# programmerjake/path-trace

Hardware: AMD Instinct MI355X
Metric: Msamples/sec at 1920x1080x1024spp; per-channel RMSE vs CPU ref (higher is better)
Workload: dtype f32; 1 GPU; C3: 1920x1080, 1024 spp, depth 8, north star: 6-sphere union/difference CSG; order=fast

## Files before the change

__graft_entry__.py:

```python
import os
import sys

ROOT = os.path.dirname(os.path.abspath(__file__))
for p in (os.path.join(ROOT, "path-trace_amd"), os.path.join(ROOT, "oracle"), os.path.join(ROOT, "tests")):
    if p not in sys.path:
        sys.path.insert(0, p)


def build() -> None:
    import build_ext
    import oracle_py
    build_ext.build()
    oracle_py.build(ref=True)
    import time
    from concurrent.futures import ProcessPoolExecutor
    start = time.time() - 1
    workers = max(1, min(8, (os.cpu_count() or 1)))
    with ProcessPoolExecutor(max_workers=workers) as ex:
        list(ex.map(_compile_job, range(len(_jobs()) + len(_test_defines()))))
    from pathtrace import _lib
    from pathtrace._lib import lib
    if not _have_gpu():
        _precompile_selftest()
    _prune_cache(start)
    print("build ok:", _lib.LIB_PATH, lib().pt_version().decode())


def _jobs():
    from pathtrace.modules import product_jobs
    jobs = product_jobs()
    try:
        import precompile_modules as test_modules
    except ImportError:
        return jobs
    jobs = jobs + test_modules.test_jobs()
    try:
        import precompile_multispan as multispan_modules
    except ImportError:
        return jobs
    jobs = jobs + multispan_modules.test_jobs()
    try:
        import precompile_lane_resume as lane_resume_modules
    except ImportError:
        return jobs
    return jobs + lane_resume_modules.test_jobs()


def _compile_job(k: int) -> None:
    import pathtrace as pt
    jobs = _jobs()
    if k >= len(jobs):
        import zoo
        from precompile_modules import TEST_DEFINES
        defs, builder, depth, ls = TEST_DEFINES[k - len(jobs)]
        os.environ["PT_DEVICE_DEFINES"] = defs
        try:
            pt.DeviceScene(zoo.build(builder), lane_scatter=ls).compile(depth)
        finally:
            del os.environ["PT_DEVICE_DEFINES"]
        return
    make, depth = jobs[k]
    obj = make()
    if depth is not None:
        obj.compile(depth)


def _test_defines():
    try:
        from precompile_modules import TEST_DEFINES
    except ImportError:
        return []
    return TEST_DEFINES


CACHE = os.path.join(ROOT, "path-trace_amd", "_jit_cache")


def _prune_cache(since: float) -> None:
    if not os.path.isdir(CACHE):
        return
    for f in os.listdir(CACHE):
        if f.endswith(".hsaco") and os.path.getmtime(os.path.join(CACHE, f)) < since:
            for ext in (".hsaco", ".hip"):
                q = os.path.join(CACHE, f[:-6] + ext)
                if os.path.exists(q):
                    os.remove(q)


def _have_gpu() -> bool:
    try:
        import torch
        return torch.cuda.device_count() > 0
    except Exception:
        return False


def _precompile_selftest() -> None:
    import ctypes
    from pathtrace import _lib
    out = (ctypes.c_uint64 * 3)()
    _lib.lib().pt_selftest_math(0, 0, 0, out)


def smoke() -> None:
    import numpy as np
    import oracle_py as O
    import pathtrace as pt
    from pathtrace import scenes
    from pathtrace.scene import to_text
    W, H, spp, depth = 24, 16, 4, 8
    root = scenes.scene_p1()
    gpu = pt.render(root, W, H, spp, depth, order="fast", device=0).reshape(-1, 3)
    ref = O.render(to_text(root, "/tmp/pt_smoke_img"), W, H, spp, depth, order=O.ORDER_FAST)
    bad = int(np.sum(gpu.view(np.uint32) != ref.view(np.uint32)))
    if bad:
        raise AssertionError("smoke: %d of %d values differ from the oracle" % (bad, gpu.size))
    rmse = np.sqrt(np.mean((gpu.astype(np.float64) - ref) ** 2, axis=0))
    print("smoke ok: %dx%d x %d spp, bit-exact vs oracle, rmse %s, mean %s" % (W, H, spp, rmse, gpu.mean(axis=0)))


if __name__ == "__main__":
    if len(sys.argv) > 1 and sys.argv[1] == "smoke":
        smoke()
    else:
        build()
```

path-trace_amd/csrc/device/pt_device.h:

```cpp
#ifndef PT_DEVICE_H
#define PT_DEVICE_H

#if defined(PT_KEPT_NORM) || defined(PT_FAST_NORM) || defined(PT_FAST_MIRRORBALL) || defined(PT_UNIT_RAY) ||        \
    defined(PT_INERT) || defined(PT_PLANE_AXIS_DARK) || defined(PT_PLANE_AXIS_DIV) || defined(PT_MERGE_FROM_SPANS) || \
    defined(PT_UNION_FUSED) || defined(PT_CTX_VGPR) || defined(PT_CLEAR_UNION) || defined(PT_LSUM_LDS) ||             \
    defined(PT_RING_SPLIT) || defined(PT_LANE_MAJOR) || defined(PT_LM_CHAINS) || defined(PT_LM_BITS) ||               \
    defined(PT_RING_FITS) || defined(PT_PASS_PAIR_FALLBACK) || defined(PT_KATT_SHORT) || defined(PT_SHORT_REM) ||     \
    defined(PT_PAD_VALU) || defined(PT_PAD_SALU) || defined(PT_NO_AXIS_SHARE) || defined(PT_FAST_LANE) ||             \
    defined(PT_RECEDE_DEAD)
#error "a retired build-time knob is defined (PT_KEPT_NORM PT_FAST_NORM PT_FAST_MIRRORBALL PT_UNIT_RAY PT_INERT PT_PLANE_AXIS_DARK PT_PLANE_AXIS_DIV PT_MERGE_FROM_SPANS PT_UNION_FUSED PT_CTX_VGPR PT_CLEAR_UNION PT_LSUM_LDS PT_RING_SPLIT PT_LANE_MAJOR PT_LM_CHAINS PT_LM_BITS PT_RING_FITS PT_PASS_PAIR_FALLBACK PT_KATT_SHORT PT_SHORT_REM PT_PAD_VALU PT_PAD_SALU PT_NO_AXIS_SHARE PT_FAST_LANE PT_RECEDE_DEAD): its arm is gone, see DESIGN.md s2, Build-time knobs that remain"
#endif

typedef unsigned long long u64;
typedef unsigned int u32;

namespace ptd
{

constexpr float EPS = 1e-3f;
constexpr float MAXV = 1e20f;
constexpr u64 LCG_MULT = 214013ull;
constexpr u64 LCG_INC = 2531011ull;

struct PtImage
// ... 1118 lines not shown
                return;
            }
        }
#endif
        typename Pln<P, O, M, AX, U>::St s;
        Pln<P, O, M, AX, U>::init(s, c, q, e);
        acc.add(s.live, s.t0, s.t1, M);
    }
    __device__ static __forceinline__ void fill(float4 *, int *, const typename Pln<P, O, M, AX, U>::Ctx &) {}
};
template <class A, class B>
struct Compact<Uni<A, B>>
{
    static constexpr bool OK = Compact<A>::OK && Compact<B>::OK;
    __device__ static __forceinline__ void run(UnionAcc &acc, u64 &m, PlaneStash &st, const typename Uni<A, B>::Ctx &c,
                                               const Ray &q, const Env &e)
    {
        Compact<A>::run(acc, m, st, c.a, q, e);
        Compact<B>::run(acc, m, st, c.b, q, e);
    }
    __device__ static __forceinline__ void fill(float4 *tab, int *mt, const typename Uni<A, B>::Ctx &c)
    {
        Compact<A>::fill(tab, mt, c.a);
        Compact<B>::fill(tab, mt, c.b);
    }
};
template <class R>
__device__ __forceinline__ int compact_first_hit(const typename R::Ctx &ctx, const Ray &q, const Env &e,
                                                 const float4 *tab, const int *mt, bool &hit, float &t, int &mat)
{
    UnionAcc acc;
    u64 m = 0ull;
    PlaneStash st;
#pragma unroll
    for (int k = 0; k < 3; k++)
        st.has[k][0] = st.has[k][1] = 0;
    Compact<R>::run(acc, m, st, ctx, q, e);
#if defined(PT_AXIS_SHARE) && PT_PLANE_PAIR
    auto unit_plane = [&](int k, int side, float num, int mat) {
        const float dk = k == 0 ? q.d.x : k == 1 ? q.d.y : q.d.z;
        const float div = side ? -dk : dk;
        const bool small = __builtin_fabsf(div) < EPS * EPS;
        const float q0 = div_core(num, q.rk[k]);
        float t = side ? -q0 : q0;
        const bool bad = !small && !(q.rkok[k] && num_ok(num));
        if (wave_any(bad)) {
            if (bad)
                t = num / div;
        }
        const bool deg = small || __builtin_fabsf(t) >= MAXV;
        const bool neg = div < 0.0f;
        acc.add((!deg || __builtin_fabsf(num) < EPS * EPS) ? 1 : 0, (!deg && neg) ? t : -MAXV,
                (!deg && !neg) ? t : MAXV, mat);
    };
#pragma unroll
    for (int k = 0; k < 3; k++) {
        if (st.has[k][0] && st.has[k][1]) {
            const float dk = k == 0 ? q.d.x : k == 1 ? q.d.y : q.d.z;
            const int side = dk < 0.0f ? 0 : 1;
            unit_plane(k, side, side ? st.num[k][1] : st.num[k][0], side ? st.mat[k][1] : st.mat[k][0]);
        } else {
            if (st.has[k][0])
                unit_plane(k, 0, st.num[k][0], st.mat[k][0]);
            if (st.has[k][1])
                unit_plane(k, 1, st.num[k][1], st.mat[k][1]);
        }
    }
#endif
    while (wave_any(m != 0ull)) {
        if (m != 0ull) {
            const int k = __builtin_ctzll(m);
            m &= m - 1ull;
            const float4 sp = tab[k];
            const float b = (sp.x * q.d.x + sp.y * q.d.y) + sp.z * q.d.z;
            const float disc = b * b - q.a * sp.w;
            const float sq = sqrt_core(disc);
            const float n0 = -b - sq, n1 = -b + sq;
            float t0 = div_core(n0, q.ra), t1 = div_core(n1, q.ra);
            if (!(q.aok && num_ok(n0) && num_ok(n1)))
                t0 = n0 / q.a, t1 = n1 / q.a;
            acc.add(1, t0, t1, mt[k]);
        }
    }
    mat = acc.bm;
    t = acc.b0;
    hit = acc.found && acc.b0 < MAXV;
    return ((!acc.found) | ((acc.b0 >= EPS) & !acc.tie)) & !acc.bad;
}

#ifndef PT_OCCLUDE
#define PT_OCCLUDE 1
#endif
template <class N>
struct Occl
{
    static constexpr bool OK = false;
};
template <int P, int O, int M>
struct Occl<Sph<P, O, M>>
{
    static constexpr bool OK = true;
    template <class SEL>
    __device__ static __forceinline__ float emis_lb(const typename Sph<P, O, M>::Ctx &, const Env &)
    {
        return SEL::take(M) ? 0.0f : __builtin_inff();
    }
    template <class SEL>
    __device__ static __forceinline__ u64 occ(const typename Sph<P, O, M>::Ctx &, V3, float, const Env &)
    {
        return 0ull;
    }
};
template <int P, int O, int M, int AX, int U>
struct Occl<Pln<P, O, M, AX, U>>
{
    static constexpr bool OK = true;
    template <class SEL>
    __device__ static __forceinline__ float emis_lb(const typename Pln<P, O, M, AX, U>::Ctx &c, const Env &e)
    {
        if constexpr (!SEL::take(M))
            return __builtin_inff();
        const float nn = __builtin_sqrtf(dot(mk(e.P[O], e.P[O + 1], e.P[O + 2]), mk(e.P[O], e.P[O + 1], e.P[O + 2])));
        return c.num <= -1e-3f ? (-c.num / nn) * 0.999f : 0.0f;
    }
    template <class SEL>
    __device__ static __forceinline__ u64 occ(const typename Pln<P, O, M, AX, U>::Ctx &c, V3 w, float g, const Env &e)
    {
        if constexpr (SEL::take(M) || AX < 0) {
            return 0ull;
        } else {
            const float na = e.P[O + (AX >> 1)];
            const float wa = (AX >> 1) == 0 ? w.x : (AX >> 1) == 1 ? w.y : w.z;
            const float lim = fmaxf(1e-4f, -c.num * g);
            return __ballot(c.num <= -1e-3f && na * wa < -lim);
        }
    }
};
template <class A, class B>
struct Occl<Uni<A, B>>
{
    static constexpr bool OK = Occl<A>::OK && Occl<B>::OK;
    template <class SEL>
    __device__ static __forceinline__ float emis_lb(const typename Uni<A, B>::Ctx &c, const Env &e)
    {
        return fminf(Occl<A>::template emis_lb<SEL>(c.a, e), Occl<B>::template emis_lb<SEL>(c.b, e));
    }
    template <class SEL>
    __device__ static __forceinline__ u64 occ(const typename Uni<A, B>::Ctx &c, V3 w, float g, const Env &e)
    {
        return Occl<A>::template occ<SEL>(c.a, w, g, e) | Occl<B>::template occ<SEL>(c.b, w, g, e);
    }
};

template <class N>
struct BFlips
{
    __device__ static constexpr int of(int) { return 0; }
};
template <class A, class B>
struct BFlips<Uni<A, B>>
{
    __device__ static constexpr int of(int prim) { return prim < A::HI ? BFlips<A>::of(prim) : BFlips<B>::of(prim); }
};
template <class A, class B>
struct BFlips<Isect<A, B>>
{
    __device__ static constexpr int of(int prim) { return prim < A::HI ? BFlips<A>::of(prim) : BFlips<B>::of(prim); }
};
template <class A, class B>
struct BFlips<Diff<A, B>>
{
    __device__ static constexpr int of(int prim) { return prim < A::HI ? BFlips<A>::of(prim) : 1 + BFlips<B>::of(prim); }
};

template <int MOFF, int IOFF, class C>
struct Xf
{
    static constexpr int LO = C::LO, HI = C::HI;
    static constexpr bool UNION_ONLY = C::UNION_ONLY;
    static constexpr bool NO_DIFF = C::NO_DIFF;
    template <class PS>
    __device__ static __forceinline__ int isect_empty(const PS &ps) { return C::isect_empty(ps); }
    struct Ctx
    {
        typename C::Ctx c;
    };
    typedef typename C::St St;
    __device__ static __forceinline__ void prep(Ctx &c, V3 o, const Env &e) { C::prep(c.c, univ(m_apply(e.P + MOFF, o)), e); }
    __device__ static __forceinline__ void prep_l(Ctx &c, V3 o, const Env &e) { C::prep_l(c.c, m_apply(e.P + MOFF, o), e); }
    __device__ static __forceinline__ void init(St &s, const Ctx &c, const Ray &q, const Env &e)
    {
        C::init(s, c.c, mkray(m_lin(e.P + MOFF, q.d)), e);
    }
    __device__ static __forceinline__ bool pull(St &s, CS &out) { return C::pull(s, out); }
    template <class PS>
    __device__ static __forceinline__ void span(PS &ps, const Ctx &c, const Ray &q, const Env &e)
    {
        C::span(ps, c.c, mkray(m_lin(e.P + MOFF, q.d)), e);
    }
    template <class PS>
    __device__ static __forceinline__ void init_ps(St &s, const PS &ps) { C::init_ps(s, ps); }
    template <class F>
    __device__ static __forceinline__ void each_pos(F &&f) { C::each_pos(f); }
    template <class SEL, class PS>
    __device__ static __forceinline__ void span_sel(PS &ps, const Ctx &c, const Ray &q, const Env &e)
    {
        C::template span_sel<SEL>(ps, c.c, mkray(m_lin(e.P + MOFF, q.d)), e);
    }
    template <class SEL, class F>
    __device__ static __forceinline__ void each_sel(F &&f) { C::template each_sel<SEL>(f); }
    template <class SEL, bool NORM>
    __device__ static __forceinline__ u64 clear_mask(const Ctx &c, const Ray &q, const Env &e)
    {
        return C::template clear_mask<SEL, false>(c.c, mkray(m_lin(e.P + MOFF, q.d)), e);
    }
    template <class SEL>
    __device__ static constexpr bool clear_ok() { return C::template clear_ok<SEL>(); }
    template <class PS>
    __device__ static __forceinline__ int fast_ok(const PS &ps) { return C::fast_ok(ps); }
    __device__ static __forceinline__ V3 normal(int prim, float t, V3 o, V3 d, const Env &e)
    {
        V3 n = C::normal(prim, t, m_apply(e.P + MOFF, o), m_lin(e.P + MOFF, d), e);
        if constexpr (!C::NO_DIFF) {
            const bool neg = BFlips<C>::of(prim) & 1;
            n = neg ? -n : n;
            n = normalize(m_lin(e.P + IOFF, n));
            return neg ? -n : n;
        }
        return normalize(m_lin(e.P + IOFF, n));
    }
    template <class SEL>
    __device__ static constexpr bool raw_ok() { return C::template nsel<SEL>() == 0; }
    template <class SEL>
    __device__ static constexpr int nsel() { return C::template nsel<SEL>(); }
    template <class SEL>
    __device__ static __forceinline__ u64 dark_mask(const Ctx &, V3, const Env &) { return ~0ull; }
    template <class SEL>
    __device__ static __forceinline__ bool dark_pre(const Ctx &, const Env &) { return true; }
};
template <int MOFF, int IOFF, class C>
struct BFlips<Xf<MOFF, IOFF, C>>
{
    __device__ static constexpr int of(int prim) { return BFlips<C>::of(prim); }
};

template <class R>
__device__ __forceinline__ bool first_hit(const typename R::Ctx &ctx, V3 d, const Env &e, float &t, u32 &ref,
                                          bool &exit_hit)
{
#ifdef PT_MERGE_STUB
    (void)ctx, (void)d, (void)e, (void)t, (void)ref, (void)exit_hit;
    return false;
#endif
    typename R::St st;
    R::init(st, ctx, mkray(d), e);
    CS s;
    while (R::pull(st, s)) {
        if (s.t0 >= MAXV)
            return false;
        if (s.t0 >= EPS) {
            t = s.t0, ref = s.r0, exit_hit = false;
            return true;
        }
        if (s.t1 >= MAXV)
            return false;
        if (s.t1 >= EPS) {
            t = s.t1, ref = s.r1, exit_hit = true;
            return true;
        }
    }
    return false;
}

template <class R, class PS>
__device__ __forceinline__ bool first_hit_ps(const PS &ps, float &t, u32 &ref, bool &exit_hit)
{
    typename R::St st;
    R::init_ps(st, ps);
    CS s;
    while (R::pull(st, s)) {
        if (s.t0 >= MAXV)
            return false;
        if (s.t0 >= EPS) {
            t = s.t0, ref = s.r0, exit_hit = false;
            return true;
        }
        if (s.t1 >= MAXV)
            return false;
        if (s.t1 >= EPS) {
            t = s.t1, ref = s.r1, exit_hit = true;
            return true;
        }
    }
    return false;
}

template <class R, class PS>
__device__ __forceinline__ int cheap_ok(const PS &ps);
template <class R, class PS>
__device__ __forceinline__ int span_first_hit(const PS &ps, bool &hit, float &t, u32 &ref, bool &exit_hit)
{
    int fok;
    if constexpr (R::NO_DIFF) {
        fok = cheap_ok<R>(ps);
        if (wave_any(!fok)) {
            if (!fok)
// ... 752 lines not shown
    const W2 b1 = lcg_step(a3), b2 = lcg_step(b1), b3 = lcg_step(b2);
    s = ((u64)b3.hi << 32) | (u64)b3.lo;
    return attempt2_draws<KR0>(a1, a2, a3, b1, b2, b3, n, kR);
}
template <bool KR0>
__device__ __forceinline__ Attempt2 attempt2_draws(W2 a1, W2 a2, W2 a3, W2 b1, W2 b2, W2 b3, V3 n, V3 kR)
{
    const f2 S = 0x1p-31f, M1 = -1.0f;
    f2 x = {(float)a1.hi, (float)b1.hi}, y = {(float)a2.hi, (float)b2.hi}, z = {(float)a3.hi, (float)b3.hi};
    x = __builtin_elementwise_fma(x, S, M1);
    y = __builtin_elementwise_fma(y, S, M1);
    z = __builtin_elementwise_fma(z, S, M1);
    const f2 vv = (x * x + y * y) + z * z;
    if (!KR0) {
        x = x + kR.x;
        y = y + kR.y;
        z = z + kR.z;
    }
#ifndef PT_HEMI_MODE
#define PT_HEMI_MODE 1
#endif
#if PT_HEMI_MODE == 1
    const f2 nw = {(n.x * x.x + n.y * y.x) + n.z * z.x, (n.x * x.y + n.y * y.y) + n.z * z.y};
#elif PT_HEMI_MODE == 2
    float vnx, vny, vnz;
    asm("v_mov_b32 %0, %1" : "=v"(vnx) : "s"(n.x));
    asm("v_mov_b32 %0, %1" : "=v"(vny) : "s"(n.y));
    asm("v_mov_b32 %0, %1" : "=v"(vnz) : "s"(n.z));
    const f2 nw = (x * vnx + y * vny) + z * vnz;
#else
    const f2 nw = (x * n.x + y * n.y) + z * n.z;
#endif
    Attempt2 r;
    r.x = x, r.y = y, r.z = z;
    const bool ba = !(vv.x > 0x1.000002p+0f), bb = !(vv.y > 0x1.000002p+0f);
    const bool ha = !(nw.x <= EPS), hb = !(nw.y <= EPS);
    const u64 BA = __ballot(ba), HA = __ballot(ha), BBm = __ballot(bb), HBm = __ballot(hb);
    r.A[0] = BA & HA, r.F[0] = BA & ~HA, r.acc[0] = ba && ha;
    r.A[1] = BBm & HBm, r.F[1] = BBm & ~HBm, r.acc[1] = bb && hb;
    return r;
}

__device__ __forceinline__ int replay(u64 A, u64 F, u64 NL, int rem, int &fails, int &reason, u64 &take)
{
    const int pa = __popcll(A), pf = __popcll(F);
    if (NL == 0ull && pa < rem && fails + pf < 1000) {
        take = A;
        if (A) {
            const int last = 63 - __builtin_clzll(A);
            fails = (last == 63) ? 0 : __popcll(F >> (last + 1));
        } else {
            fails += pf;
        }
        return 63;
    }
    const int nl = NL ? __builtin_ctzll(NL) : 64;
    const int pos_rem = (pa >= rem) ? nth_set_bit(A, rem) : 64;
    int pos_abort = 64;
    if (fails + pf >= 1000) {
        int fc = fails;
        for (int l = 0; l < 64; l++) {
            if (l == nl || l == pos_rem)
                break;
            if ((A >> l) & 1ull)
                fc = 0;
            else if ((F >> l) & 1ull) {
                if (++fc == 1000) {
                    pos_abort = l;
                    break;
                }
            }
        }
    }
    if (pos_abort < 64 && pos_abort < nl && pos_abort < pos_rem) {
        reason = B_ABORT;
        take = A & ((1ull << pos_abort) - 1ull);
        return pos_abort;
    }
    if (nl < 64 && nl <= pos_rem) {
        reason = B_NONLEAF;
        take = A & ((1ull << nl) - 1ull);
        return nl;
    }
    if (pos_rem < 64) {
        reason = B_DONE;
        take = (pos_rem == 63) ? A : (A & ((2ull << pos_rem) - 1ull));
        return pos_rem;
    }
    take = A;
    if (A) {
        const int last = 63 - __builtin_clzll(A);
        fails = (last == 63) ? 0 : __popcll(F >> (last + 1));
    } else {
        fails += pf;
    }
    return 63;
}

template <class S, bool STRICT, bool DEFERRED, bool KR0>
__device__ __forceinline__ int burst_t(const Env &e, Rng &rng, const u64 *__restrict__ jump, const JumpLds &J,
                                       const WaveLds &L, Frame &f, Frame &child, Counters &cnt)
{
    float4 *const ring = L.ring;
    unsigned char *const slowq = L.slowq, *const midq = L.midq;
    constexpr bool LANE_REMAT = PT_LANE_REMAT < 0 ? S::Root::NO_DIFF : PT_LANE_REMAT != 0;
    const int lane_reg = threadIdx.x & 63;
#define lane (LANE_REMAT ? lane_id() : lane_reg)
    const bool LSUM_LDS = L.lsum != nullptr;
    const V3 hit = univ(f.hit), n = univ(f.n), rc = univ(f.rc);
    const float sc = unif(f.sc), strength = unif(f.strength), add = unif(f.add);
    const int depth = uni(f.depth), N = uni(f.N);
    const int i = uni(f.i);
    V3 retval = univ(f.retval);
    const V3 kR = univ((1.0f / sc - 1.0f) * univ(f.refl));
    const float sNa = unif((strength / (float)N) * add);
    const float aN = unif(add / (float)N);
    const float abs_rc = unif(length(rc));
    const bool child_leaf_depth = depth - 1 <= 0;
    auto lane_state = [&]() {
        u64 jA, jG;
        jread(J.j3, lane, jA, jG);
        return jA * rng.st + jG;
    };
    const u64 A64 = jump[128], g64inc = jump[129] * LCG_INC;
    const u64 Afull = jump[128 * PT_KATT], gfullinc = jump[128 * PT_KATT + 1] * LCG_INC;
    int fails = 0, reason = -1;
    LdsBox<typename S::Root::Ctx> *const cxp = (LdsBox<typename S::Root::Ctx> *)L.ctx;
    typename S::Root::Ctx c0;
    S::Root::prep(c0, hit, e);
    lds_put(*cxp, c0);
    if constexpr (PT_SPH_COMPACT && Compact<typename S::Root>::OK)
        Compact<typename S::Root>::fill(L.stab, L.smat, c0);
    int npos = 0, nkeep = 0, keep_sum = 0, nzc = 0, f_n = 0, s_head = 0, s_n = 0, s_first = 0;
    int m_head = 0, m_n = 0, m_first = 0;
    V3 lsum = mk(0.0f, 0.0f, 0.0f);
    if (LSUM_LDS)
        L.lsum[lane] = L.lsum[64 + lane] = L.lsum[128 + lane] = 0.0f;
    int fast_on = 1, clear_on = 1;
    constexpr bool CLEAR = S::Root::template clear_ok<Emissive<S>>() && !S::Root::UNION_ONLY;
    constexpr bool RAW = DEFERRED && !STRICT && S::Root::template raw_ok<Emissive<S>>();
    const bool wfin = __builtin_fabsf(rc.x) < 1e37f && __builtin_fabsf(rc.y) < 1e37f && __builtin_fabsf(rc.z) < 1e37f;
    const u64 raw_mask =
        uni_mask((KR0 || length(kR) < 64.0f) && wfin && S::Root::template dark_pre<Emissive<S>>(c0, e));
#if PT_OCCLUDE
    constexpr bool OCC = RAW && Occl<typename S::Root>::OK;
#else
    constexpr bool OCC = false;
#endif
    float occ_g = __builtin_inff();
    if constexpr (OCC) {
        const float te = fminf(Occl<typename S::Root>::template emis_lb<Emissive<S>>(c0, e), 1e19f);
        const float bw = (KR0 ? 1.0f : 1.0f + length(kR)) * 1.0001f;
        occ_g = unif(te > 0.0f ? bw * 1.001f / te : __builtin_inff());
    }
    auto dark = [&](V3 wn) -> u64 {
        u64 d = S::Root::template dark_mask<Emissive<S>>(c0, wn, e);
        if constexpr (OCC)
            d |= Occl<typename S::Root>::template occ<Emissive<S>>(c0, wn, occ_g, e);
        return d & raw_mask;
    };
    const bool short_nd = !DEFERRED && EPS < 0.99f * (sNa * abs_rc);
    auto slot_pos = [&](unsigned char v) { return keep_sum + ((int)(v - keep_sum) & (PT_RCAP - 1)); };
    PT_CNT(cnt, 0, 1);
    for (;;) {
        PT_CNT(cnt, 1, 1);
        const bool room = PT_RCAP - (nkeep - keep_sum) >= 64;
        if (reason < 0 && room) {
            PT_T0(tg);
            PT_MARK(13);
            int rem = N - (i + npos);
            const int katt = (rem <= 24 || (!DEFERRED && short_nd)) ? PT_KATT : PT_KATT;
            int free_slots = PT_RCAP - (nkeep - keep_sum);
#ifdef PT_ROOM_CAP
            free_slots = min(free_slots, PT_ROOM_CAP);
#endif
            int ta = 0, tk = 0;
            u64 nlor = 0ull, Alast = 0ull, Flast = 0ull;
            const int slot_end = nkeep + free_slots;
            auto write_attempt = [&](u64 A, u64 kp, V3 wn, float factor) {
                const int slot = mbcnt(kp, nkeep + tk);
                if (in_mask(kp & __ballot(slot < slot_end)))
                    ring[slot & (PT_RCAP - 1)] = make_float4(wn.x, wn.y, wn.z, factor);
                ta += __popcll(A);
                tk += __popcll(kp);
            };
            int fails_lm = 0;
            if constexpr (DEFERRED) {
                u64 jA, jG;
                jread(J.j24, lane, jA, jG);
                const u64 s_lane = jA * rng.st + jG;
                u32 abits = 0u, fbits = 0u, kbits = 0u;
                u64 sk = s_lane;
#pragma unroll
                for (int k = 0; k < PT_KATT; k += 2) {
                    const Attempt2 ap = attempt2_chain<KR0>(sk, n, kR);
#pragma unroll
                    for (int h = 0; h < 2; h++) {
                        const V3 wn = h ? mk(ap.x.y, ap.y.y, ap.z.y) : mk(ap.x.x, ap.y.x, ap.z.x);
                        u64 D = 0ull;
                        if (RAW)
                            D = dark(wn);
                        abits = shl_lane_bit(abits, ap.A[h]);
                        fbits = shl_lane_bit(fbits, ap.F[h]);
                        kbits = shl_lane_bit(kbits, ap.A[h] & ~D);
                    }
                }
                const u32 tfl = (u32)__popc(fbits & ((abits & (0u - abits)) - 1u));
                const u32 pk = (u32)__popc(abits) | ((u32)__popc(kbits) << 10) | (tfl << 20);
                const u32 incl = wave_incl_scan(pk), excl = incl - pk;
                const u32 tot = (u32)__builtin_amdgcn_readlane((int)incl, 63);
                ta = (int)(tot & 0x3FFu);
                tk = (int)((tot >> 10) & 0x3FFu);
                const u64 Aor = __ballot(abits != 0u);
                if (Aor) {
                    const int L = 63 - __builtin_clzll(Aor);
                    fails_lm = (int)(tot >> 20) - (int)((u32)__builtin_amdgcn_readlane((int)excl, L) >> 20);
                } else {
                    fails_lm = fails + (int)(tot >> 20);
                }
                int slot = nkeep + (int)((excl >> 10) & 0x3FFu);
                auto put = [&](u32 kb, bool check) {
                    for (; kb != 0u;) {
                        const int c = __builtin_clz(kb);
                        if (!check || slot < slot_end) {
                            float4 *r = &ring[slot & (PT_RCAP - 1)];
                            __builtin_memcpy(r, &s_lane, 8);
                            r->z = __int_as_float(c - (32 - PT_KATT));
                        }
                        slot++;
                        kb ^= 0x80000000u >> c;
                    }
                };
                if (tk <= free_slots)
                    put(kbits, false);
                else
                    put(kbits, true);
            } else {
                u64 sk = lane_state();
#pragma unroll
                for (int k = 0; k < PT_KATT; k++) {
                    if (k >= katt)
                        break;
                    if (k)
                        sk = A64 * sk + g64inc;
                    const Attempt at = attempt<DEFERRED, KR0>(sk, n, kR, sc, sNa, abs_rc, child_leaf_depth);
                    write_attempt(at.A, at.A, at.wn, at.factor);
                    nlor |= at.NL;
                    if (k == katt - 1)
                        Alast = at.A, Flast = at.F;
                }
            }
            PT_ACC(cnt, 1, tg);
#ifdef PT_FULL_STATS
            cadd(cnt.rounds, 1u);
#endif
            if (DEFERRED && KR0)
                PT_MARK(14);
            int m;
            int np, nk;
            if (nlor == 0ull && ta < rem && tk <= free_slots && fails <= 999 - 64 * katt && (DEFERRED || Alast != 0ull)) {
                if (DEFERRED) {
                    fails = fails_lm;
                } else {
                    const int last = 63 - __builtin_clzll(Alast);
                    fails = (last == 63) ? 0 : __popcll(Flast >> (last + 1));
                }
                m = 64 * katt;
                np = ta;
                nk = tk;
            } else {
                PT_COLD();
                Attempt at[PT_KATT];
                u64 Dm[PT_KATT];
                {
                    u64 sk = lane_state();
#pragma unroll
                    for (int k = 0; k < PT_KATT; k++) {
                        if (k)
                            sk = A64 * sk + g64inc;
                        at[k] = attempt<DEFERRED, KR0>(sk, n, kR, sc, sNa, abs_rc, child_leaf_depth);
                        Dm[k] = 0ull;
                        if (RAW)
                            Dm[k] = dark(at[k].wn);
                    }
                }
                m = 0;
                np = nk = 0;
                bool cut = false;
#pragma unroll
                for (int k = 0; k < PT_KATT; k++) {
                    if (reason < 0 && !cut && k < katt) {
                        u64 take = 0ull;
                        const int fails_in = fails;
                        const int c = replay(at[k].A, at[k].F, at[k].NL, rem, fails, reason, take);
                        m = 64 * k + c + 1;
                        rem -= __popcll(at[k].A);
                        u64 kp = take & ~Dm[k];
                        if (__popcll(kp) > free_slots) {
                            const int pos = nth_set_bit(kp, free_slots + 1);
                            const u64 pre = (1ull << pos) - 1ull;
                            take &= pre;
                            kp &= pre;
                            const u64 ca = at[k].A & pre;
                            if (ca) {
                                const int last = 63 - __builtin_clzll(ca);
                                fails = __popcll(at[k].F & pre & ~((2ull << last) - 1ull));
// ... 61 lines not shown
                }
                return false;
            }
            PrimSpans<S::Root::HI> ps;
            PT_MARK(9);
            S::Root::span(ps, ctx, mkray_unit(dir), e);
            PT_MARK(10);
            if constexpr (S::Root::UNION_ONLY) {
                bool fh;
                float t;
                int mat;
                fok = union_first_hit<typename S::Root>(ps, fh, t, mat);
                PT_MARK(11);
                if (fok) {
                    V3 col = mk(0, 0, 0);
                    if (fh)
                        col = S::emis(mat, hit + t * dir, e);
                    PT_MARK(12);
                    const V3 term = ((aN * en.w) * rc) * col;
                    ring[pos & (PT_RCAP - 1)] = make_float4(term.x, term.y, term.z, 0.0f);
                    return true;
                }
                return false;
            }
            if constexpr (S::Root::NO_DIFF) {
                fok = cheap_ok<typename S::Root>(ps);
            } else {
                fok = S::Root::fast_ok(ps);
            }
            PT_MARK(11);
            if (fok) {
                float t = 0.0f;
                int mat = 0;
                V3 col = mk(0, 0, 0);
                if (fast_first_hit<typename S::Root>(ps, t, mat))
                    col = S::emis(mat, hit + t * dir, e);
                PT_MARK(12);
                const V3 term = ((aN * en.w) * rc) * col;
                ring[pos & (PT_RCAP - 1)] = make_float4(term.x, term.y, term.z, 0.0f);
                return true;
            }
            return false;
        };
        auto enqueue = [&](unsigned char *q, int head, int &qn, int &qfirst, u64 SM, int pos0, int pos) {
            if ((SM >> lane) & 1ull)
                q[mbcnt(SM, head + qn) & (PT_SCAP - 1)] = (unsigned char)pos;
            if (qn == 0 && SM)
                qfirst = pos0 + __builtin_ctzll(SM);
            qn += __popcll(SM);
        };
        for (;;) {
            if (s_n > 0 && (s_n >= 64 || (drain && m_n == 0 && f_n == 0))) {
                PT_T0(tc);
                const int cs = s_n < 64 ? s_n : 64;
                PT_CNT(cnt, 4, 1);
                PT_CNT(cnt, 7, cs);
                if (lane < cs) {
                    const int pos = slot_pos(slowq[(s_head + lane) & (PT_SCAP - 1)]);
                    const float4 en = ring[pos & (PT_RCAP - 1)];
                    const V3 dir = mk(en.x, en.y, en.z);
                    const typename S::Root::Ctx ctx = lds_get(*cxp);
                    float t;
                    u32 ref;
                    bool ex;
                    V3 col = mk(0, 0, 0);
#ifndef PT_SLOW_STUB
                    if (first_hit<typename S::Root>(ctx, dir, e, t, ref, ex))
                        col = S::emis(ref_mat(ref), hit + t * dir, e);
#else
                    (void)ctx, (void)t, (void)ref, (void)ex;
#endif
                    const V3 term = ((aN * en.w) * rc) * col;
                    ring[pos & (PT_RCAP - 1)] = make_float4(term.x, term.y, term.z, 0.0f);
                }
                s_head += cs;
                s_n -= cs;
                if (s_n)
                    s_first = slot_pos(uni(slowq[s_head & (PT_SCAP - 1)]));
                PT_ACC(cnt, 3, tc);
                continue;
            }
            if (CLEAR && m_n > 0 && (m_n >= 64 || (drain && f_n == 0))) {
                PT_T0(tb);
                const int cm = m_n < 64 ? m_n : 64;
                int slow = 0, pos = 0;
                if (lane < cm) {
                    pos = slot_pos(midq[(m_head + lane) & (PT_SCAP - 1)]);
                    const float4 en = ring[pos & (PT_RCAP - 1)];
                    slow = (!fast_on || !fast_lane(pos, en)) ? 1 : 0;
                }
                const u64 SM = __ballot(slow);
                const int p0 = uni(__builtin_amdgcn_readlane(pos, SM ? __builtin_ctzll(SM) : 0));
                if ((SM >> lane) & 1ull)
                    slowq[mbcnt(SM, s_head + s_n) & (PT_SCAP - 1)] = (unsigned char)pos;
                if (s_n == 0 && SM)
                    s_first = p0;
                s_n += __popcll(SM);
                cadd(cnt.slow, (u32)__popcll(SM));
                if (fast_on && 4 * __popcll(SM) > 3 * cm)
                    fast_on = 0;
                m_head += cm;
                m_n -= cm;
                if (m_n)
                    m_first = slot_pos(uni(midq[m_head & (PT_SCAP - 1)]));
                PT_ACC(cnt, 2, tb);
                continue;
            }
            if (f_n > 0 && (f_n >= 64 || drain)) {
                PT_T0(tb);
                const int cf = f_n < 64 ? f_n : 64;
                const int pos0 = nkeep - f_n;
                const int pos = pos0 + lane;
                PT_CNT(cnt, 3, 1);
                PT_CNT(cnt, 6, cf);
                int park = 0;
                if (lane < cf) {
                    float4 en = ring[pos & (PT_RCAP - 1)];
                    if (DEFERRED) {
                        u64 st;
                        __builtin_memcpy(&st, &en, 8);
                        {
                            u64 jA, jG;
                            jread(J.j3, __float_as_int(en.z), jA, jG);
                            st = jA * st + jG;
                        }
                        const W2 s1 = lcg_step({(u32)st, (u32)(st >> 32)}), s2 = lcg_step(s1), s3 = lcg_step(s2);
                        V3 w = mk(u11(s1.hi), u11(s2.hi), u11(s3.hi));
                        if (!KR0)
                            w = w + kR;
                        const V3 nd = KR0 ? cnormalize_kept(w) : cnormalize(w);
                        en = make_float4(nd.x, nd.y, nd.z,
                                         KR0 ? 1.0f - (1.0f - dot(nd, n)) : 1.0f - (1.0f - dot(nd, n)) * sc);
                    }
                    if constexpr (CLEAR) {
                        park = 1;
                        if (clear_on) {
                            PT_MARK(16);
                            const V3 dir = mk(en.x, en.y, en.z);
                            const typename S::Root::Ctx ctx = lds_get(*cxp);
                            const Ray q = mkray_unit(dir);
                            const u64 CM = S::Root::template clear_mask<Emissive<S>, true>(ctx, q, e);
                            PrimSpans<S::Root::HI> ps;
                            S::Root::template span_sel<Emissive<S>>(ps, ctx, q, e);
                            if (((CM >> lane) & 1ull) && sel_ok<typename S::Root, Emissive<S>>(ps)) {
                                float t = 0.0f;
                                int mat = 0;
                                V3 col = mk(0, 0, 0);
                                if (sel_first_hit<typename S::Root, Emissive<S>>(ps, t, mat))
                                    col = S::emis(mat, hit + t * dir, e);
                                const V3 term = ((aN * en.w) * rc) * col;
                                ring[pos & (PT_RCAP - 1)] = make_float4(term.x, term.y, term.z, 0.0f);
                                park = 0;
                            }
                            PT_MARK(17);
                        }
                        if (DEFERRED && park)
                            ring[pos & (PT_RCAP - 1)] = en;
                    } else {
                        if (!fast_on || !fast_lane(pos, en)) {
                            park = 2;
                            if (DEFERRED)
                                ring[pos & (PT_RCAP - 1)] = en;
                        }
                    }
                }
                if constexpr (CLEAR) {
                    const u64 MM = __ballot(park == 1);
                    enqueue(midq, m_head, m_n, m_first, MM, pos0, pos);
                    cadd(cnt.mid, (u32)__popcll(MM));
                    if (clear_on && 4 * __popcll(MM) > 3 * cf)
                        clear_on = 0;
                } else {
                    const u64 SM = __ballot(park == 2);
                    enqueue(slowq, s_head, s_n, s_first, SM, pos0, pos);
                    cadd(cnt.slow, (u32)__popcll(SM));
                    if (fast_on && 4 * __popcll(SM) > 3 * cf)
                        fast_on = 0;
                }
                f_n -= cf;
                PT_ACC(cnt, 2, tb);
                continue;
            }
            break;
        }
        PT_T0(ts);
        {
            int resolved = nkeep - f_n;
            if (m_n)
                resolved = min(resolved, m_first);
            if (s_n)
                resolved = min(resolved, s_first);
            while (resolved - keep_sum >= 64 || (drain && resolved > keep_sum)) {
                const int c = min(64, resolved - keep_sum);
                PT_CNT(cnt, 5, 1);
                V3 t = mk(0.0f, 0.0f, 0.0f);
                if (lane < c) {
                    const float4 tv = ring[(keep_sum + lane) & (PT_RCAP - 1)];
                    t = mk(tv.x, tv.y, tv.z);
                }
                if (STRICT) {
                    for (int j = 0; j < c; j++)
                        retval = retval + mk(rdlane(t.x, j), rdlane(t.y, j), rdlane(t.z, j));
                } else {
                    const u64 nz = __ballot(t.x != 0.0f) | __ballot(t.y != 0.0f) | __ballot(t.z != 0.0f);
                    const int pnz = __popcll(nz);
                    const int k = mask_sel(nz, mbcnt(nz, nzc), mbcnt(~nz, nzc + pnz));
                    const int to = (k & 63) << 2;
                    t = mk(__int_as_float(__builtin_amdgcn_ds_permute(to, __float_as_int(t.x))),
                           __int_as_float(__builtin_amdgcn_ds_permute(to, __float_as_int(t.y))),
                           __int_as_float(__builtin_amdgcn_ds_permute(to, __float_as_int(t.z))));
                    if (LSUM_LDS) {
                        float *const q = L.lsum;
                        const int l = lane;
                        q[l] = q[l] + t.x, q[64 + l] = q[64 + l] + t.y, q[128 + l] = q[128 + l] + t.z;
                    } else {
                        lsum = lsum + t;
                    }
                    nzc += pnz;
                }
                keep_sum += c;
            }
        }
        PT_ACC(cnt, 4, ts);
        if (final)
            break;
    }
    if (!STRICT && npos > 0) {
        if (LSUM_LDS) {
            const int l = lane;
            lsum = mk(L.lsum[l], L.lsum[64 + l], L.lsum[128 + l]);
        }
        retval = wave_tree_sum3_add(lsum, retval);
    }
    cadd(cnt.leaf, (u32)npos);
    cadd(cnt.dark, (u32)(npos - nkeep));
    f.retval = retval;
    f.i = i + npos;
    return reason;
}
#undef lane

#ifndef PT_REACH_PRUNE
#define PT_REACH_PRUNE 1
#endif
template <class S>
struct Reach
{
    static constexpr int kr = PT_REACH_PRUNE ? S::kr_reach : 3;
    static constexpr bool all_leaf = PT_REACH_PRUNE ? S::bursts_all_leaf : false;
};
template <class S, bool STRICT>
__device__ __forceinline__ int burst(const Env &e, Rng &rng, const u64 *__restrict__ jump, const JumpLds &jl,
                                     const WaveLds &L, Frame &f, Frame &child, Counters &cnt)
{
    [[maybe_unused]] bool deferred = true;
    if constexpr (!Reach<S>::all_leaf) {
        const float sNa = unif((unif(f.strength) / (float)uni(f.N)) * unif(f.add));
        const float abs_rc = unif(length(univ(f.rc)));
        deferred = uni(f.depth) - 1 <= 0 || (sNa * abs_rc * 1.01f < EPS);
    }
    PT_T0(t0);
    int r;
    if constexpr (!Reach<S>::all_leaf)
        if (!deferred) {
            r = burst_t<S, STRICT, false, false>(e, rng, jump, jl, L, f, child, cnt);
            PT_ACC(cnt, 5, t0);
            return r;
        }
    if constexpr (Reach<S>::kr == 1)
        r = burst_t<S, STRICT, true, true>(e, rng, jump, jl, L, f, child, cnt);
    else if constexpr (Reach<S>::kr == 2)
        r = burst_t<S, STRICT, true, false>(e, rng, jump, jl, L, f, child, cnt);
    else if (unif(f.sc) == 1.0f)
        r = burst_t<S, STRICT, true, true>(e, rng, jump, jl, L, f, child, cnt);
    else
        r = burst_t<S, STRICT, true, false>(e, rng, jump, jl, L, f, child, cnt);
    PT_ACC(cnt, 5, t0);
    return r;
}

enum { PH_ENTER, PH_SETUP, PH_LOOP, PH_RETURN };
enum { RS_REFRACT, RS_SCATTER };

#ifndef PT_ZERO_CHILD
#define PT_ZERO_CHILD 1
#endif
__device__ __forceinline__ bool zero_child(V3 w, float cstr, int cdep, V3 part)
{
    const u32 wz = (__float_as_uint(w.x) | __float_as_uint(w.y) | __float_as_uint(w.z)) << 1;
    auto ok = [](float v) { return v == v && __float_as_uint(v) != 0x80000000u; };
    return wz == 0u && (cdep <= 0 || cstr < EPS) && ok(part.x) && ok(part.y) && ok(part.z);
}

struct CamHit
{
    int hit;
    float t;
    u32 ref;
    int ex;
};

__device__ __forceinline__ V3 camera_dir(const PtLaunch &lp, int pix, Rng &rng)
{
    const int px = pix % lp.gw, py = pix / lp.gw;
    float x = 2.0f * ((float)px + u01(rng_next(rng))) / (float)lp.W - 1.0f;
    float y = 1.0f - 2.0f * ((float)py + u01(rng_next(rng))) / (float)lp.H;
// ... 1475 lines not shown
```

Before: 211.2 Msamples/s.

## Add inside-sphere zero-contribution test to resolve parked CSG samples early

Adds an Inside<> template over the CSG tree that runs a conservative analytic test on sphere/difference/union nodes. It proves that a sample ray starts inside a non-emissive solid, so its contribution is zero. Such samples are written as zero to the ring and unparked on the clear path, instead of being deferred to the full mid-queue trace. This adds per-lane sphere evaluations to the clear branch and relies on margin-based conservativeness for exactness. The build script also orders compile jobs so that new test modules compile.

```diff
diff --git a/__graft_entry__.py b/__graft_entry__.py
--- a/__graft_entry__.py
+++ b/__graft_entry__.py
@@ -17,7 +17,7 @@
     start = time.time() - 1
     workers = max(1, min(8, (os.cpu_count() or 1)))
     with ProcessPoolExecutor(max_workers=workers) as ex:
-        list(ex.map(_compile_job, range(len(_jobs()) + len(_test_defines()))))
+        list(ex.map(_compile_job, _job_order()))
     from pathtrace import _lib
     from pathtrace._lib import lib
     if not _have_gpu():
@@ -43,7 +43,21 @@
         import precompile_lane_resume as lane_resume_modules
     except ImportError:
         return jobs
-    return jobs + lane_resume_modules.test_jobs()
+    jobs = jobs + lane_resume_modules.test_jobs()
+    return jobs + _inside_zero_jobs()
+
+
+def _inside_zero_jobs():
+    try:
+        import precompile_inside_zero as inside_zero_modules
+    except ImportError:
+        return []
+    return inside_zero_modules.test_jobs()
+
+
+def _job_order():
+    n, tail = len(_jobs()), len(_inside_zero_jobs())
+    return list(range(n, n + len(_test_defines()))) + list(range(n - tail, n)) + list(range(n - tail))
 
 
 def _compile_job(k: int) -> None:
diff --git a/path-trace_amd/csrc/device/pt_device.h b/path-trace_amd/csrc/device/pt_device.h
--- a/path-trace_amd/csrc/device/pt_device.h
+++ b/path-trace_amd/csrc/device/pt_device.h
@@ -1294,6 +1294,127 @@
     }
 };
 
+#ifndef PT_INSIDE_ZERO
+#define PT_INSIDE_ZERO 1
+#endif
+struct InsideG
+{
+    float mg, xmin;
+};
+struct InsideV
+{
+    float bmin, bmax, xbest, xlo;
+};
+template <class N>
+struct Inside
+{
+    template <class SEL>
+    __device__ static constexpr bool ok() { return false; }
+    template <class SEL>
+    __device__ static constexpr bool sph_only() { return false; }
+};
+template <int P, int O, int M>
+struct Inside<Sph<P, O, M>>
+{
+    template <class SEL>
+    __device__ static constexpr bool ok() { return !SEL::take(M); }
+    template <class SEL>
+    __device__ static constexpr bool sph_only() { return !SEL::take(M); }
+    template <class SEL>
+    __device__ static __forceinline__ float emis_lb(const typename Sph<P, O, M>::Ctx &, const Env &)
+    {
+        return __builtin_inff();
+    }
+    __device__ static __forceinline__ float far2(const typename Sph<P, O, M>::Ctx &c, const Env &e)
+    {
+        return c.c + 2.0f * e.P[O + 3];
+    }
+    __device__ static __forceinline__ InsideV eval(const typename Sph<P, O, M>::Ctx &c, const Ray &q, const InsideG &g)
+    {
+        const float b = dot(c.omc, q.d);
+        const float disc = b * b - q.a * c.c;
+        const float sq = __builtin_amdgcn_sqrtf(disc);
+        const bool dead = disc <= EPS;
+        InsideV v;
+        v.bmin = dead ? __builtin_inff() : -b - sq;
+        v.bmax = dead ? -__builtin_inff() : -b + sq;
+        v.xbest = v.bmax > g.xmin ? v.bmax : -__builtin_inff();
+        v.xlo = v.bmin;
+        return v;
+    }
+};
+template <int P, int O, int M, int AX, int U>
+struct Inside<Pln<P, O, M, AX, U>>
+{
+    template <class SEL>
+    __device__ static constexpr bool ok() { return true; }
+    template <class SEL>
+    __device__ static constexpr bool sph_only() { return false; }
+    template <class SEL>
+    __device__ static __forceinline__ float emis_lb(const typename Pln<P, O, M, AX, U>::Ctx &c, const Env &e)
+    {
+        return Occl<Pln<P, O, M, AX, U>>::template emis_lb<SEL>(c, e);
+    }
+    __device__ static __forceinline__ float far2(const typename Pln<P, O, M, AX, U>::Ctx &, const Env &) { return 0.0f; }
+    __device__ static __forceinline__ InsideV eval(const typename Pln<P, O, M, AX, U>::Ctx &, const Ray &, const InsideG &)
+    {
+        return {-__builtin_inff(), __builtin_inff(), -__builtin_inff(), 0.0f};
+    }
+};
+#define PTD_INSIDE_COMMON(NODE)                                                                                  \
+    template <class SEL>                                                                                         \
+    __device__ static constexpr bool sph_only()                                                                  \
+    {                                                                                                            \
+        return Inside<A>::template sph_only<SEL>() && Inside<B>::template sph_only<SEL>();                       \
+    }                                                                                                            \
+    template <class SEL>                                                                                         \
+    __device__ static __forceinline__ float emis_lb(const typename NODE<A, B>::Ctx &c, const Env &e)             \
+    {                                                                                                            \
+        return fminf(Inside<A>::template emis_lb<SEL>(c.a, e), Inside<B>::template emis_lb<SEL>(c.b, e));        \
+    }                                                                                                            \
+    __device__ static __forceinline__ float far2(const typename NODE<A, B>::Ctx &c, const Env &e)                \
+    {                                                                                                            \
+        return fmaxf(Inside<A>::far2(c.a, e), Inside<B>::far2(c.b, e));                                          \
+    }
+template <class A, class B>
+struct Inside<Uni<A, B>>
+{
+    template <class SEL>
+    __device__ static constexpr bool ok() { return Inside<A>::template ok<SEL>() && Inside<B>::template ok<SEL>(); }
+    PTD_INSIDE_COMMON(Uni)
+    __device__ static __forceinline__ InsideV eval(const typename Uni<A, B>::Ctx &c, const Ray &q, const InsideG &g)
+    {
+        const InsideV a = Inside<A>::eval(c.a, q, g), b = Inside<B>::eval(c.b, q, g);
+        const bool ta = a.xbest >= b.xbest;
+        return {-__builtin_inff(), __builtin_inff(), ta ? a.xbest : b.xbest, ta ? a.xlo : b.xlo};
+    }
+};
+template <class A, class B>
+struct Inside<Diff<A, B>>
+{
+    template <class SEL>
+    __device__ static constexpr bool ok() { return sph_only<SEL>(); }
+    PTD_INSIDE_COMMON(Diff)
+    __device__ static __forceinline__ InsideV eval(const typename Diff<A, B>::Ctx &c, const Ray &q, const InsideG &g)
+    {
+        const InsideV a = Inside<A>::eval(c.a, q, g), b = Inside<B>::eval(c.b, q, g);
+        const bool pass = a.xbest > b.bmax + g.mg && b.bmin > a.xlo + g.mg;
+        return {-__builtin_inff(), __builtin_inff(), pass ? a.xbest : -__builtin_inff(), fmaxf(a.xlo, b.bmax)};
+    }
+};
+template <class A, class B>
+struct Inside<Isect<A, B>>
+{
+    template <class SEL>
+    __device__ static constexpr bool ok() { return sph_only<SEL>(); }
+    PTD_INSIDE_COMMON(Isect)
+    __device__ static __forceinline__ InsideV eval(const typename Isect<A, B>::Ctx &, const Ray &, const InsideG &)
+    {
+        return {-__builtin_inff(), __builtin_inff(), -__builtin_inff(), 0.0f};
+    }
+};
+#undef PTD_INSIDE_COMMON
+
 template <class N>
 struct BFlips
 {
@@ -2352,6 +2473,21 @@
         const float te = fminf(Occl<typename S::Root>::template emis_lb<Emissive<S>>(c0, e), 1e19f);
         const float bw = (KR0 ? 1.0f : 1.0f + length(kR)) * 1.0001f;
         occ_g = unif(te > 0.0f ? bw * 1.001f / te : __builtin_inff());
+    }
+#if PT_INSIDE_ZERO
+    constexpr bool INS = CLEAR && !STRICT && Inside<typename S::Root>::template ok<Emissive<S>>();
+#else
+    constexpr bool INS = false;
+#endif
+    InsideG ins_g = {0.0f, 0.0f};
+    int ins_on = 0;
+    if constexpr (INS) {
+        const float te = fminf(Inside<typename S::Root>::template emis_lb<Emissive<S>>(c0, e), 1e15f);
+        const float g2 = 2.02f * Inside<typename S::Root>::far2(c0, e);
+        const float g = __builtin_sqrtf(g2);
+        ins_on = uni((wfin && te > 0.0f && g2 < te * te) ? 1 : 0);
+        ins_g.mg = unif(1e-5f * g);
+        ins_g.xmin = unif(EPS * 1.001f + 1e-5f * g);
     }
     auto dark = [&](V3 wn) -> u64 {
         u64 d = S::Root::template dark_mask<Emissive<S>>(c0, wn, e);
@@ -2719,6 +2855,15 @@
                                 ring[pos & (PT_RCAP - 1)] = make_float4(term.x, term.y, term.z, 0.0f);
                                 park = 0;
                             }
+                            if constexpr (INS) {
+                                if (ins_on) {
+                                    const InsideV iv = Inside<typename S::Root>::eval(ctx, q, ins_g);
+                                    if (park && iv.xbest > 0.0f) {
+                                        ring[pos & (PT_RCAP - 1)] = make_float4(0.0f, 0.0f, 0.0f, 0.0f);
+                                        park = 0;
+                                    }
+                                }
+                            }
                             PT_MARK(17);
                         }
                         if (DEFERRED && park)
```

After: 234.1 Msamples/s (median of 6 runs). 10.9% higher.
